# lukasc-ch/CBinfer

Measured on AMD Instinct MI355X. Metric: frames/sec + effective GFLOP/s vs dense, scene-labeling CNN 480x320 @10% change, higher is better.
Workload: dtype f32-equivalent: f32 tensors, every operand as three bf16 terms (24 bits, exact), six products on the bf16 MFMA, f32 accumulate; 1 GPU; sceneLabeling CBConv2d coarse-grained fp32, synthetic 480x320 seq @10% change (32x32 re-drawn blocks), experiment 6, one sequence per GPU; sequences_per_gpu=1, launch=program

## Files before the change

### cbinfer_amd/_lib.py

```python
import ctypes
import os

_PKG = os.path.dirname(os.path.abspath(__file__))
LIB_PATH = os.path.join(_PKG, "libcbinfer_hip.so")

CB_F32 = 0
CB_F16 = 1
CB_F32S = 2

_vp, _i, _l, _f = ctypes.c_void_p, ctypes.c_int, ctypes.c_long, ctypes.c_float


class SplitSeq(ctypes.Structure):
    _fields_ = [("input", _vp), ("state", _vp), ("splitState", _vp), ("frameMasks", _vp), ("producerMask", _vp),
                ("output", _vp), ("idxOut", _vp), ("countOut", _vp), ("rangeFlag", _vp), ("maskCopy", _vp),
                ("delta", _vp), ("reluOut", _vp)]


_sp = ctypes.POINTER(SplitSeq)


class TailSeq(ctypes.Structure):
    _fields_ = [("input", _vp), ("changeList", _vp), ("countDev", _vp), ("output", _vp)]

# ... 146 lines not shown
    "cbinfer_rowconv_prep_weights": (_i, [_vp, _vp, _i, _i, _i, _i, _vp]),
    "cbinfer_conv_changed_rows": (_i, [_vp, _vp, _vp, _vp, _vp, _vp, _vp, _i, _i, _i, _i, _i, _i, _i, _vp]),
    "cbinfer_change_detection_bits_pooled": (_i, [_vp, _i, _i, _vp, _vp, _vp, _i, _i, _i, _i, _i, _f, _i, _vp]),
    "cbinfer_cbconv2d_forward_rows": (_i, [_vp, _vp, _i, _i, _vp, _vp, _vp, _vp, _vp, _vp, _vp, _vp, _i, _i, _i,
                                           _i, _i, _i, _f, _i, _i, _i, _vp]),
    "cbinfer_cbconv2d_forward_blocks": (_i, [_vp, _vp, _i, _i, _vp, _vp, _vp, _vp, _vp, _vp, _vp, _vp, _i, _i,
                                             _i, _i, _i, _i, _f, _i, _i, _i, _vp]),
    "cbinfer_blockconv_supported": (_i, [_i, _i, _i, _i]),
    "cbinfer_blockconv_prepared_bytes": (_l, [_i, _i, _i, _i]),
    "cbinfer_blockconv_prep_weights": (_i, [_vp, _vp, _i, _i, _i, _i, _vp]),
    "cbinfer_conv_changed_blocks": (_i, [_vp, _vp, _vp, _vp, _vp, _vp, _vp, _i, _i, _i, _i, _i, _i, _i, _vp]),
    "cbinfer_change_detection_bits_batched": (_i, [_vpp, _vpp, _vpp, _i, _i, _i, _i, _i, _i, _f, _i, _vp]),
    "cbinfer_conv_changed_rows_batched": (_i, [_vpp, _vpp, _vpp, _vpp, _vpp, _i, _vp, _vp, _i, _i, _i, _i, _i, _i, _i,
                                               _vp]),
    "cbinfer_tail1x1_batched": (_i, [_tp, _i, _i, _vp, _vp, _vp, _vp, _i, _i, _i, _i, _i, _i, _i, _vp]),
    "cbinfer_split_supported": (_i, [_i, _i, _i, _i]),
    "cbinfer_split_max_sequences": (_i, []),
    "cbinfer_split_max_mask_words": (_l, [_i]),
    "cbinfer_split_state_bytes": (_l, [_i, _i, _i, _i, _i]),
    "cbinfer_split_prepared_bytes": (_l, [_i, _i, _i, _i]),
    "cbinfer_split_workspace_bytes": (_l, [_i, _i, _i, _i, _i, _i, _i]),
    "cbinfer_split_prep_weights": (_i, [_vp, _vp, _i, _i, _i, _i, _i, _i, _f, _vp]),
    "cbinfer_split_state_init": (_i, [_vp, _i, _i, _i, _i, _i, _vp]),
    "cbinfer_split_state_rebuild": (_i, [_vp, _vp, _i, _i, _i, _i, _i, _vp, _vp]),
    "cbinfer_split3_state_bytes": (_l, [_i, _i, _i, _i, _i]),
    "cbinfer_split3_prepared_bytes": (_l, [_i, _i, _i, _i]),
    "cbinfer_split3_prep_weights": (_i, [_vp, _vp, _i, _i, _i, _i, _i, _i, _vp]),
    "cbinfer_split3_state_init": (_i, [_vp, _i, _i, _i, _i, _i, _vp]),
    "cbinfer_split3_state_rebuild": (_i, [_vp, _vp, _i, _i, _i, _i, _i, _vp]),
    "cbinfer_split_detect": (_i, [_sp, _i, _i, _i, _i, _i, _i, _i, _i, _i, _f, _vp]),
    "cbinfer_split_conv": (_i, [_sp, _i, _vp, _vp, _i, _i, _i, _i, _i, _i, _f, _i, _vp, _i, _vp]),
    "cbinfer_split_forward": (_i, [_sp, _i, _i, _i, _i, _vp, _vp, _i, _i, _i, _i, _i, _i, _f, _f, _i, _vp, _vp]),
    "cbinfer_split_next_supported": (_i, [_i, _i, _i, _i, _i, _i, _ndp]),
    "cbinfer_split_conv_next": (_i, [_sp, _i, _vp, _vp, _i, _i, _i, _i, _i, _i, _f, _i, _vp, _ndp, _vp]),
    "cbinfer_split_refresh_supported": (_i, [_i, _i, _i, _i, _i, _i]),
    "cbinfer_split_conv_refresh": (_i, [_sp, _i, _vp, _vp, _i, _i, _i, _i, _i, _i, _f, _i, _vp, _srp, _vp]),
    "cbinfer_split_conv_next_refresh": (_i, [_sp, _i, _vp, _vp, _i, _i, _i, _i, _i, _i, _f, _i, _vp, _ndp, _srp, _vp]),
    "cbinfer_split_forward_next": (_i, [_sp, _i, _i, _i, _i, _vp, _vp, _i, _i, _i, _i, _i, _i, _f, _f, _i, _vp, _ndp,
                                        _vp]),
    "cbinfer_split_forward_fg": (_i, [_sp, _i, _i, _i, _i, _vp, _i, _i, _i, _i, _i, _i, _f, _f, _vp, _vp]),
    "cbinfer_hsplit_supported": (_i, [_i, _i, _i, _i]),
    "cbinfer_hsplit_max_mask_words": (_l, [_i]),
    "cbinfer_hsplit_state_bytes": (_l, [_i, _i, _i, _i, _i]),
    "cbinfer_hsplit_prepared_bytes": (_l, [_i, _i, _i, _i]),
    "cbinfer_hsplit_workspace_bytes": (_l, [_i, _i, _i, _i, _i, _i]),
    "cbinfer_hsplit_prep_weights": (_i, [_vp, _vp, _i, _i, _i, _i, _i, _i, _vp]),
    "cbinfer_hsplit_state_init": (_i, [_vp, _i, _i, _i, _i, _i, _vp]),
    "cbinfer_hsplit_state_rebuild": (_i, [_vp, _vp, _i, _i, _i, _i, _i, _vp]),
    "cbinfer_hsplit_forward": (_i, [_vp, _vp, _i, _i, _i, _vp, _vp, _vp, _vp, _vp, _vp, _vp, _vp, _vp, _vp, _i, _i, _i,
                                    _i, _i, _i, _f, _i, _i, _vp, _vp]),
    "cbinfer_hsplit_group_workspace_bytes": (_l, [_i, _i, _i, _i, _i, _i, _i]),
    "cbinfer_hsplit_forward_group": (_i, [_hlp, _i, _i, _i, _i, _i, _i, _i, _i, _i, _i, _vp, _vp]),
    "cbinfer_split_forward_tail": (_i, [_sp, _i, _i, _i, _i, _vp, _vp, _i, _i, _i, _i, _i, _i, _f, _f, _i, _vp, _i,
                                        _stp, _vp]),
    "cbinfer_split_forward_fg_tail": (_i, [_sp, _i, _i, _i, _i, _vp, _i, _i, _i, _i, _i, _i, _f, _f, _vp, _stp, _vp]),
    "cbinfer_split_tail_supported": (_i, [_i, _i, _i, _i, _i, _i]),
    "cbinfer_split_conv_tail": (_i, [_sp, _i, _vp, _vp, _i, _i, _i, _i, _i, _i, _f, _i, _vp, _i, _stp, _vp]),
    "cbinfer_rowpairs_supported": (_i, [_i, _i, _i, _i, _i, _i]),
    "cbinfer_conv_changed_rowpairs": (_i, [_vp, _vp, _vp, _vp, _vp, _vp, _vp, _i, _i, _i, _i, _i, _i, _i, _ndp, _vp]),
    "cbinfer_conv_changed_rowpairs_batched": (_i, [_psp, _i, _vp, _vp, _i, _i, _i, _i, _i, _i, _i, _ndp, _vp]),
    "cbinfer_conv_rowpairs_detect": (_i, [_vp, _vp, _vp, _vp, _vp, _vp, _i, _i, _i, _i, _i, _i, _f, _i, _ndp, _vp]),
    "cbinfer_refresh_state": (_i, [_vp, _vp, _i, _i, _i, _f, _vp]),
    "cbinfer_cbconv2d_forward_rowpairs": (_i, [_vp, _vp, _vp, _vp, _vp, _vp, _vp, _vp, _i, _i, _i, _i, _i, _i, _f, _i,
                                               _ndp, _vp]),
    "cbinfer_frame_mask_copy_offset": (_l, [_i, _i]),
    "cbinfer_concat_channels": (_i, [_vpp, ctypes.POINTER(ctypes.c_int32), _i, _vp, _l, _i, _vp]),
# ... 124 lines not shown
```

### cbinfer_amd/csrc/cb_split.hip

```cpp
#include <stdlib.h>

#include <type_traits>

#include "cb_common.h"

#ifdef CBS_STAMP
__device__ unsigned long long cbs_stamp_buf[4 * 2048 * 16];
#define CB_TAIL_STAMP(i)                                                                 \
    do {                                                                                 \
        if (threadIdx.x == 0 && blockIdx.x < 2048)                                       \
            cbs_stamp_buf[(2 * 2048 + blockIdx.x) * 16 + (i)] = __builtin_amdgcn_s_memrealtime(); \
    } while (0)
#define CBS_DET_STAMP(i)                                                                                            \
    do {                                                                                                            \
        const unsigned wg = blockIdx.y * gridDim.x + blockIdx.x;                                                    \
        if (POOL && threadIdx.x == 0 && blockIdx.z == 0 && wg < 2048)                                               \
            cbs_stamp_buf[(3 * 2048 + wg) * 16 + (i)] = __builtin_amdgcn_s_memrealtime();                            \
    } while (0)
#else
#define CBS_DET_STAMP(i)
#endif
#include "cb_tail_core.h"
#include "cb_split_common.h"

// ... 266 lines not shown
#define CBH_NEXT CBINFER_HNEXT_MAX
struct CbhNext {
    _Float16* state;
    char* S;
    unsigned long long* masks;
    int kHH, kWH, Wp, rec, padY, padXL;
    float th;
    int pad_;
};
struct CbhLayer {
    const char* A;
    const _Float16* bias;
    int K, relu, nNext, pad_;
    CbhNext next[CBH_NEXT];
};
struct CbhExt {
    CbhLayer L[CBH_GROUP];
    int slabCap1;
    int pad_;
};
struct CbsNoExt {};
struct CbsWinExt {
    float* nstate;
    char* nS;
    unsigned long long* nmasks;
    int* nflag;
    int H2, W2, wpr2, kHH, kWH, Wp, rec, padY, padXL, planes;
    float th;
    unsigned long long magicW2;
    const float* sideFrame;
    float* sideState;
    int sideC, sideHW;
    float sideTh;
};
template <int AR>
struct CbsExtOf {
    typedef CbsNoExt type;
};
template <>
struct CbsExtOf<1> {
    typedef CbhExt type;
};
template <>
struct CbsExtOf<3> {
    typedef CbsWinExt type;
};
struct CbsSideExt {
    const float* sideFrame;
    float* sideState;
    int sideC, sideHW;
    float sideTh;
};
template <>
struct CbsExtOf<4> {
    typedef CbsSideExt type;
};

__device__ __forceinline__ void cbh_or_dilated(unsigned long long* masks, int y, int x, int H, int W, int wpr, int kHH,
                                               int kWH) {
    const int lo = max(x - kWH, 0), hi = min(x + kWH, W - 1);
    const int w0 = lo >> 6, w1 = hi >> 6;
    const unsigned long long m0 = (~0ull << (lo & 63)) & (w1 == w0 ? (~0ull >> (63 - (hi & 63))) : ~0ull);
    const unsigned long long m1 = ~0ull >> (63 - (hi & 63));
    for (int yy = max(y - kHH, 0); yy <= min(y + kHH, H - 1); ++yy) {
        atomicOr(&masks[(long)yy * wpr + w0], m0);
        if (w1 != w0) atomicOr(&masks[(long)yy * wpr + w1], m1);
// ... 27 lines not shown

template <int OFF>
__device__ __forceinline__ halfx8 cbs_lds_read16(unsigned addr) {
    halfx8 v;
    asm volatile("ds_read_b128 %0, %1 offset:%2" : "=v"(v) : "v"(addr), "n"(OFF));
    return v;
}

__device__ __forceinline__ int cbs_div(int x, unsigned long long magic) {
    return (int)(((unsigned long long)(unsigned)x * magic) >> 32);
}

template <int BM, int BN, int WM, int WN, int PRE_CAP, bool MASK_LDS, int RING, int AR = 0>
__global__ __launch_bounds__(64 * WM * WN) void cbs_conv_kernel(CbsParams p, typename CbsExtOf<AR>::type ext) {
    constexpr bool HALF = AR == 1, X3 = AR == 2 || AR == 3 || AR == 4, WIN = AR == 3, SIDE = AR == 3 || AR == 4;
    if (HALF && p.upstream && *p.upstream == 0) {
        if (blockIdx.x == 0 && threadIdx.x == 0) {
            p.seq[0].countOut[0] = 0;
            if (p.info) p.info[CBS_INFO_SK] = 1;
        }
        return;
    }
    cb_touch_kernarg<sizeof(CbsParams) + (HALF ? sizeof(CbhExt) : (WIN ? sizeof(CbsWinExt) : (SIDE ? sizeof(CbsSideExt) : 0)))>();
    constexpr int NW = WM * WN, NT = 64 * NW;
    constexpr int TN = BN / WN / 32;
    static_assert(BM == 32 * WM, "one 32-row tile per wave");
    constexpr int PB = X3 ? 192 : 128;
    constexpr int ABLK = BM * PB / 1024, BBLK = BN * PB / 1024;
    constexpr int APW = ABLK / NW, BPW = BBLK / NW;
    static_assert(APW * NW == ABLK && BPW * NW == BBLK && APW >= 1 && BPW >= 1, "DMA blocks must deal evenly");
    constexpr int DPW = APW + BPW;
    constexpr int A_BYTES = BM * PB, B_BYTES = BN * PB, STAGE = A_BYTES + B_BYTES;
    constexpr int TILE = BM * BN;
    __shared__ __attribute__((aligned(1024))) char ring[RING * STAGE];
    __shared__ int s_pre[PRE_CAP + 1];
    __shared__ unsigned long long s_mask[MASK_LDS ? PRE_CAP : 1];
    __shared__ const unsigned long long* s_maskPtr[CBS_MAXSEQ];
    __shared__ int s_wsum[NW];
    __shared__ int s_tilePix[BN];
    __shared__ float s_bias[BM];
    __shared__ unsigned s_nchg[HALF ? CBH_NEXT * (BN / 32) : 1];
    __shared__ int s_preW[WIN ? PRE_CAP / 2 + 2 : 1];
    __shared__ int s_tileAny[WIN ? BN : 1];
    __shared__ int s_winPos[WIN ? BN / 4 : 1];
    __shared__ unsigned s_wchg;
    __shared__ unsigned long long s_wsum64[WIN ? 64 * WM * WN / 64 : 1];
    static_assert(!WIN || (BN / WN / 32 == 1 && MASK_LDS), "window order: one column tile per wave, the mask words in LDS");

    const int t = threadIdx.x;
    const int lane = t & 63, wave = __builtin_amdgcn_readfirstlane(t >> 6);
    const int wm = wave % WM, wn = wave / WM;
    const int l31 = lane & 31, h = lane >> 5;
    const int MW = p.maskWords, MT = p.KP / BM;
#ifdef CBS_STAMP
    bool cbs_first = true;
#endif
    CBS_STAMP_AT(0);
    CBS_STAMP_AT(6);

    __shared__ int s_seqN[CBS_MAXSEQ], s_seqRank[CBS_MAXSEQ], s_seqTile[CBS_MAXSEQ + 1], s_exact[CBS_MAXSEQ];
    int flagv = 0;
    static_assert(NT >= CBS_MAXSEQ, "one thread per sequence");
    if (p.nSeq == 1) {
        if (t == 0) {
            const int* rf = p.seq[0].rangeFlag;
            s_maskPtr[0] = p.seq[0].masks;
            if (rf) flagv = *rf;
// ... 252 lines not shown
        p.info[CBS_INFO_SK] = SK;
        p.info[CBS_INFO_MT] = MT;
        p.info[2] = p.nSeq;
        for (int q = 0; q < CBS_MAXSEQ; ++q) {
            p.info[CBS_INFO_TP + q] = q < p.nSeq ? s_seqTile[q + 1] - s_seqTile[q] : 0;
            p.info[CBS_INFO_TP + CBS_MAXSEQ + q] = q < p.nSeq ? s_seqN[q] : 0;
        }
        if constexpr (HALF) {
#pragma unroll
            for (int u = 0; u < CBH_GROUP; ++u) p.info[CBS_INFO_CH + u] = chQ[u];
        }
    }

    const int aRecords = (int)min(p.aBytes, (long)0x7fffffff);
    const cb_const_int* stageOff = (const cb_const_int*)p.stageOff;
    const int HW = p.H * p.W;
    const float lo2 = 1.0f / CBS_LO;

    static_assert(APW == (X3 ? 3 : 2) && BPW == APW, "four (x3: six) DMA instructions per wave and stage");
    int aRead[4];
#pragma unroll
    for (int e = 0; e < 4; ++e) {
        const int b = wm * 4 + e;
        aRead[e] = X3 ? (2 * wm) * 6144 + lane * 16 : (b / APW) * 4096 + (b % APW) * 1024 + lane * 16;
    }
    int bRead[TN];
#pragma unroll
    for (int j = 0; j < TN; ++j) {
        const int n = (wn * TN + j) * 32 + l31, c = n >> 3;
        if (X3)
            bRead[j] = (n >> 4) * 6144 + 3072 + (n & 15) * 64 + ((h ^ ((n >> 2) & 3)) << 4);
        else
            bRead[j] = (c / BPW) * 4096 + (APW + c % BPW) * 1024 + (n & 7) * 128 + ((h ^ ((n >> 1) & 7)) << 4);
    }

    for (int it = blockIdx.x; it < items; it += gridDim.x) {
        int d = cbs_div(it, p.magicMT), mt = it - d * MT;
        int slice = d & (SK - 1), ptg = SK == 1 ? d : d >> chShift;
        int q = 0, N = totAll, rb = 0, tile0 = 0;
        int CHi = CH, chShiftI = chShift;
        if constexpr (HALF) {
            static_assert(CBH_GROUP == 2, "two item ranges");
            q = (p.nSeq > 1 && it >= itemBase[1]) ? 1 : 0;
            const int local = it - (q ? itemBase[1] : 0);
            CHi = q ? chQ[CBH_GROUP - 1] : chQ[0];
            chShiftI = CHi >= 16 ? 4 : (CHi >= 8 ? 3 : 2);
            d = cbs_div(local, p.magicMT), mt = local - d * MT;
            slice = SK == 1 ? 0 : d & (CHi - 1);
            ptg = SK == 1 ? d : d >> chShiftI;
            if (p.nSeq > 1) {
                N = __builtin_amdgcn_readfirstlane(s_seqN[q]), rb = __builtin_amdgcn_readfirstlane(s_seqRank[q]);
            }
        } else if (p.nSeq > 1) {
            for (int u = 1; u < p.nSeq; ++u)
                if (ptg >= s_seqTile[u]) q = u;
            q = __builtin_amdgcn_readfirstlane(q);
            N = __builtin_amdgcn_readfirstlane(s_seqN[q]), rb = __builtin_amdgcn_readfirstlane(s_seqRank[q]);
            tile0 = __builtin_amdgcn_readfirstlane(s_seqTile[q]);
        }
        const int n0 = (ptg - tile0) * BN, m0 = mt * BM;
        const char* Aq = p.A;
        const float* biasq = p.bias;
        int Kq = p.K, reluq = p.relu, nNext = 0;
        if constexpr (HALF) {
            Aq = ext.L[q].A, biasq = (const float*)ext.L[q].bias, Kq = ext.L[q].K, reluq = ext.L[q].relu;
            nNext = __builtin_amdgcn_readfirstlane(ext.L[q].nNext);
// ... 410 lines not shown
        typedef std::integral_constant<int, 8> R8;
#define CBS_STEP3A(S, FCUR, FNEXT)                                                         \
        do {                                                                               \
            CBS_SB();                                                                      \
            mma3(KS0(), FCUR, 0, 1); CBS_SB(); read1(KS1(), P0(), (S), FNEXT); read1(KS1(), P3(), (S), FNEXT); CBS_SB(); \
            mma3(KS0(), FCUR, 1, 2); CBS_SB(); read1(KS1(), P1(), (S), FNEXT); read1(KS1(), P4(), (S), FNEXT); CBS_SB(); \
            mma3(KS0(), FCUR, 2, 3); CBS_SB(); read1(KS1(), P2t(), (S), FNEXT); read1(KS1(), P5(), (S), FNEXT); CBS_SB(); \
            mma3(KS0(), FCUR, 3, 4); CBS_SB(); read1(KS1(), R6(), (S), FNEXT); CBS_SB();   \
            mma3(KS0(), FCUR, 4, 5); CBS_SB(); read1(KS1(), R7(), (S), FNEXT); CBS_SB();   \
            mma3(KS0(), FCUR, 5, 6); CBS_SB(); read1(KS1(), R8(), (S), FNEXT); CBS_SB();   \
            mma3(KS0(), FCUR, 6, NM3);                                                     \
            waitFrags(FNEXT);                                                              \
        } while (0)
#define CBS_STEP3B(WAITN, S, FCUR, FNEXT)                                                  \
        do {                                                                               \
            asm volatile("s_waitcnt vmcnt(%0)" ::"n"(WAITN) : "memory");                  \
            __builtin_amdgcn_s_barrier();                                                  \
            CBS_SB();                                                                      \
            issue((S) + RING, true);                                                       \
            CBS_SB();                                                                      \
            mma3(KS1(), FCUR, 0, 1); CBS_SB();                                             \
            read1(KS0(), P0(), (S) + 1, FNEXT); read1(KS0(), P3(), (S) + 1, FNEXT); CBS_SB(); issuePart(P0()); CBS_SB(); \
            mma3(KS1(), FCUR, 1, 2); CBS_SB();                                             \
            read1(KS0(), P1(), (S) + 1, FNEXT); read1(KS0(), P4(), (S) + 1, FNEXT); CBS_SB(); issuePart(P1()); CBS_SB(); \
            mma3(KS1(), FCUR, 2, 3); CBS_SB();                                             \
            read1(KS0(), P2t(), (S) + 1, FNEXT); read1(KS0(), P5(), (S) + 1, FNEXT); CBS_SB(); issuePart(P2t()); CBS_SB(); \
            mma3(KS1(), FCUR, 3, 4); CBS_SB(); read1(KS0(), R6(), (S) + 1, FNEXT); CBS_SB(); issuePart(P3()); CBS_SB(); \
            mma3(KS1(), FCUR, 4, 5); CBS_SB(); read1(KS0(), R7(), (S) + 1, FNEXT); CBS_SB(); issuePart(P4()); CBS_SB(); \
            mma3(KS1(), FCUR, 5, 6); CBS_SB(); read1(KS0(), R8(), (S) + 1, FNEXT); CBS_SB(); issuePart(P5()); CBS_SB(); \
            mma3(KS1(), FCUR, 6, NM3);                                                     \
            waitFrags(FNEXT);                                                              \
        } while (0)

        constexpr bool NEXT_REGS = HALF && TN == 1;
        _Float16 hv16[NEXT_REGS ? 16 : 1], sv16[NEXT_REGS ? CBH_NEXT : 1][NEXT_REGS ? 16 : 1];
        if constexpr (NEXT_REGS) {
            if (nNext > 0 && SK == 1) {
                const int pixLd = max(s_tilePix[wn * 32 + l31], 0);
                const int nx2 = nNext > 1 ? 1 : 0;
                const int mb0 = m0 + wm * 32 + 4 * h;
#pragma unroll
                for (int r = 0; r < 16; ++r) {
                    const long o = (long)min(mb0 + 8 * (r >> 2) + (r & 3), Kq - 1) * HW + pixLd;
                    sv16[0][r] = ext.L[q].next[0].state[o];
                    if (CBH_NEXT > 1) sv16[CBH_NEXT > 1 ? 1 : 0][r] = ext.L[q].next[nx2].state[o];
                }
            }
        }
        float oldv[WIN ? 16 : 1], nsv[WIN ? 4 : 1];
        int anyPos = -1, wPos = -1;
        if constexpr (WIN) {
            const int nl = wn * 32 + l31;
            anyPos = s_tileAny[nl], wPos = s_winPos[nl >> 2];
            const int aLd = max(anyPos, 0), wLd = max(wPos, 0);
            const long H2W2 = (long)ext.H2 * ext.W2;
            const float* oq = p.seq[0].out;
            if (__builtin_amdgcn_ballot_w64(anyPos >= 0 && s_tilePix[nl] < 0) != 0ull) {
#pragma unroll
                for (int r = 0; r < 16; ++r) {
                    const int m = min(wm * 32 + (r & 3) + 8 * (r >> 2) + 4 * h, Kq - 1);
                    oldv[r] = oq[(long)m * HW + aLd];
                }
            } else {
#pragma unroll
                for (int r = 0; r < 16; ++r) oldv[r] = 0.f;
            }
            const int c0 = wm * 32 + 8 * (nl & 3) + 4 * h;
#pragma unroll
            for (int e = 0; e < 4; ++e) nsv[e] = ext.nstate[(long)min(c0 + e, Kq - 1) * H2W2 + wLd];
        }
        Frags F0, F1;
        CBS_STAMP_AT(2);
#pragma unroll
        for (int i = 0; i < RING; ++i) issue(sBeg + i);
        asm volatile("s_waitcnt vmcnt(%0)" ::"n"((RING - 1) * DPW) : "memory");
        __builtin_amdgcn_s_barrier();
        __builtin_amdgcn_sched_barrier(0);
        if constexpr (X3) {
            readA3(KS0(), sBeg, F0);
#pragma unroll
            for (int j = 0; j < TN; ++j) readB3(KS0(), sBeg, F0, j);
        } else {
            readFrags(sBeg, F0);
        }
        waitFrags(F0);
        if (t < BM) s_bias[t] = biasv;
        CBS_STAMP_AT(3);
        int s = sBeg;
        if constexpr (X3) {
            for (int c = c0; c < c1; ++c) {
                const int cEnd = chunkBeg(c + 1);
                for (; s < cEnd; ++s) {
                    CBS_STEP3A(s, F0, F1);
                    CBS_STEP3B((RING - 2) * DPW, s, F1, F0);
                }
                if (c + 1 < c1) fold();
            }
        }
        if constexpr (!X3) {
            for (int c = c0; c < c1; ++c) {
                const int cEnd = chunkBeg(c + 1);
                for (; s + 1 < cEnd; s += 2) {
                    CBS_STEP((RING - 2) * DPW, true, s, F0, F1);
                    CBS_STEP((RING - 2) * DPW, true, s + 1, F1, F0);
                }
                if (c + 1 < c1) fold();
            }
            if (s < sEnd) CBS_STEP((RING - 2) * DPW, true, s, F0, F1);
        }
        asm volatile("s_waitcnt vmcnt(0)" ::: "memory");
#undef CBS_STEP
#undef CBS_STEP3A
#undef CBS_STEP3B
#undef CBS_SB
        __builtin_amdgcn_sched_barrier(0);
        CBS_STAMP_AT(4);
        CBS_STAMP_AT(7);

        float* out = p.seq[q].out;
        int accum;
        float* reluPlane;
        {
            const char* ka = (const char*)__builtin_amdgcn_kernarg_segment_ptr();
            asm volatile("" : "+s"(ka));
            const CbsParams* pp = (const CbsParams*)ka;
            accum = pp->accumulate;
            reluPlane = accum ? pp->seq[q].reluOut : nullptr;
        }
        if (CBS_DBGBIT(32)) continue;
        if (SK > 1) {
            float4* slab = (float4*)p.slabs + (long)it * (TILE / 4);
#pragma unroll
            for (int j = 0; j < TN; ++j) {
                const int nl = (wn * TN + j) * 32 + l31;
#pragma unroll
                for (int r4 = 0; r4 < 4; ++r4) {
                    const int mq = wm * 8 + 2 * r4 + h;
                    slab[mq * BN + nl] = make_float4(comb(j, 4 * r4), comb(j, 4 * r4 + 1), comb(j, 4 * r4 + 2),
                                                     comb(j, 4 * r4 + 3));
                }
            }
            CBS_STAMP_AT(5);
#ifdef CBS_STAMP
            cbs_first = false;
// ... 746 lines not shown
        CB_REQUIRE(seqs[q].input && seqs[q].state && seqs[q].splitState && seqs[q].frameMasks);
        a.seq[q].in = seqs[q].input;
        a.seq[q].state = seqs[q].state;
        a.seq[q].S = (char*)seqs[q].splitState;
        a.seq[q].masks = (unsigned long long*)seqs[q].frameMasks;
        a.seq[q].prodMask = (pooled && !fg) ? (const unsigned long long*)seqs[q].producerMask : nullptr;
        a.seq[q].rangeFlag = x3 ? nullptr : seqs[q].rangeFlag;
        a.seq[q].delta = seqs[q].delta;
        if (fg) CB_REQUIRE(seqs[q].delta != nullptr);
    }
    a.W = W, a.H = H, a.C = C, a.kHH = (kH - 1) / 2, a.kWH = (kW - 1) / 2;
    a.wpr = cbinfer_mask_words_per_row(W), a.pH = pH, a.pW = pW;
    a.Wp = g.Wp, a.rec = g.rec, a.padY = g.padY, a.padXL = g.padXL;
    a.words = cbinfer_mask_words(H, W);
    a.th = threshold;
    a.copyAll = ((mode >> 1) & 1) | fg;
    a.fg = fg;
    dim3 grid(a.wpr, H, nSeq), block(64 * (C / 4));
    if (pooled)
        hipLaunchKernelGGL(cbs_detect_kernel<true>, grid, block, 0, (hipStream_t)stream, a);
    else
        hipLaunchKernelGGL(cbs_detect_kernel<false>, grid, block, 0, (hipStream_t)stream, a);
    return cb_launch_status();
}

static int cbs_detect_mode(int mode, float weightScale) {
    return (mode & ~CBINFER_SPLIT_X3) | (weightScale == 0.f ? CBINFER_SPLIT_X3 : 0);
}

static bool cbs_next_supported(int C, int K, int kH, int kW, int H, int W, const cbNextDetect* next) {
    if (!next || !cbs_supported(C, K, kH, kW) || K > 64 || K % 16 != 0 || !cbs_supported(K, 1, next->kH, next->kW)) return false;
    if (cbs_geom(C, H, W, kH, kW, 3).nStages >= 48) return false;
    if (!((next->H == H / 2 || next->H == (H + 1) / 2) && (next->W == W / 2 || next->W == (W + 1) / 2))) return false;
    if (next->arith != 0 && next->arith != 1) return false;
    const long MW = cbinfer_mask_words(H, W), EU = (long)((H + 1) / 2) * cbinfer_mask_words_per_row(W);
    if (MW > CBS_PRE_SMALL || 2 * EU + 2 > CBS_PRE_SMALL + 1 || EU + 1 > CBS_PRE_SMALL / 2 + 2) return false;
    const CbsGeom g2 = cbs_geom(K, next->H, next->W, next->kH, next->kW, next->arith ? 3 : 2);
    return (long)g2.Hp * g2.Wp * g2.rec < (1l << 31) && (long)H * W < (1l << 20);
}

static bool cbs_refresh_supported(int C, int K, int kH, int kW, int H, int W) {
    return cbs_supported(C, K, kH, kW) && K <= 64 && cbs_geom(C, H, W, kH, kW, 3).nStages < 48 &&
           cbinfer_mask_words(H, W) <= CBS_PRE_SMALL;
}

static int cbs_split_conv(const cbSplitSeq* seqs, int nSeq, const void* prepared, const float* bias, int C, int H,
                          int W, int K, int kH, int kW, float weightScale, int relu, void* workspace, int forceSplit,
                          const CbsTailArgs* tail, cbStream_t stream, int accumulate = 0,
                          const cbNextDetect* next = nullptr, const cbSideRefresh* side = nullptr) {
    if (workspace == nullptr && cbs_supported(C, K, kH, kW) && cbs_geom(C, H, W, kH, kW).nStages >= 48)
        return CB_ERR_BADARG;
    CB_REQUIRE(seqs && nSeq >= 1 && nSeq <= CBS_MAXSEQ && prepared && H > 0 && W > 0 && weightScale >= 0.f);
    if (!cbs_supported(C, K, kH, kW)) return CB_ERR_UNSUPPORTED;
    const bool x3 = weightScale == 0.f;
    const CbsGeom g = cbs_geom(C, H, W, kH, kW, x3 ? 3 : 2);
    const int KP = cbs_kp(K), BM = cbs_bm(K);
    const long MW = cbinfer_mask_words(H, W);
    if ((long)nSeq * MW > (BM >= 128 ? CBS_PRE_BIG : CBS_PRE_MID) || (long)g.Hp * g.Wp * g.rec >= (1l << 31) ||
        (long)H * W * W >= (1l << 32))
        return CB_ERR_UNSUPPORTED;
    CbsParams p;
    for (int q = 0; q < nSeq; ++q) {
        CB_REQUIRE(seqs[q].splitState && seqs[q].output && seqs[q].frameMasks && seqs[q].idxOut && seqs[q].countOut);
        p.seq[q].S = (const char*)seqs[q].splitState;
        p.seq[q].state = accumulate ? seqs[q].delta : seqs[q].state;
        p.seq[q].reluOut = accumulate ? seqs[q].reluOut : nullptr;
        p.seq[q].rangeFlag = (p.seq[q].state && !x3) ? seqs[q].rangeFlag : nullptr;
        p.seq[q].out = seqs[q].output;
        p.seq[q].masks = (unsigned long long*)seqs[q].frameMasks;
        p.seq[q].listOut = seqs[q].idxOut;
        p.seq[q].countOut = seqs[q].countOut;
        p.seq[q].maskCopy = (unsigned long long*)seqs[q].maskCopy;
    }
    p.nSeq = nSeq;
    p.aBytes = (long)g.nStages * (KP / 32) * (x3 ? 6144 : 4096);
    p.A = (const char*)prepared;
    p.stageOff = (const int*)((const char*)prepared + p.aBytes);
    p.wPlain = x3 ? nullptr : (const float*)((const char*)prepared + cbs_plain_offset(p.aBytes, g.nStages));
    p.bias = bias;
    p.relu = relu;
    cbs_fill_params(p, g, K, KP, BM, H, W, MW, workspace, cbs_slab_capacity(nSeq, H, W, K));
    p.outScale = x3 ? 1.0f : 1.0f / (weightScale * CBS_XSCALE);
    p.forceSK = forceSplit;
    p.accumulate = accumulate;
    p.halfOut = 0;
    p.upstream = nullptr;
    p.maxChunks = CBS_CHUNKS;
#ifdef CBS_DBG
    if (const char* e = getenv("CBINFER_SPLIT_DBG")) p.dbg = atoi(e);
#endif
    hipStream_t s = (hipStream_t)stream;
    if (side && side->frame && !next) {
        if (!cbs_refresh_supported(C, K, kH, kW, H, W) || nSeq != 1 || !x3 || accumulate || tail) return CB_ERR_UNSUPPORTED;
        CbsSideExt e;
        const int st = cbs_fill_side(e, side);
        if (st != CB_OK) return st;
        return cbs_launch_conv<64, 64, 2, 2, CBS_PRE_SMALL, true, 5, 4>(p, 1, nullptr, s, e);
    }
    if (next) {
        if (!cbs_next_supported(C, K, kH, kW, H, W, next) || nSeq != 1 || !x3 || accumulate || tail) return CB_ERR_UNSUPPORTED;
        CB_REQUIRE(next->state && next->splitState && next->frameMasks);
        const CbsGeom g2 = cbs_geom(K, next->H, next->W, next->kH, next->kW, next->arith ? 3 : 2);
        CbsWinExt e;
        e.nstate = next->state, e.nS = (char*)next->splitState, e.nmasks = (unsigned long long*)next->frameMasks;
        e.nflag = next->arith ? nullptr : next->rangeFlag;
        e.H2 = next->H, e.W2 = next->W, e.wpr2 = cbinfer_mask_words_per_row(next->W);
        e.kHH = (next->kH - 1) / 2, e.kWH = (next->kW - 1) / 2;
        e.Wp = g2.Wp, e.rec = g2.rec, e.padY = g2.padY, e.padXL = g2.padXL, e.planes = g2.planes;
        e.th = next->threshold;
        e.magicW2 = (1ull << 32) / (unsigned long long)next->W + 1ull;
        e.sideFrame = nullptr, e.sideState = nullptr, e.sideC = 0, e.sideHW = 0, e.sideTh = 0.f;
        if (side && side->frame) {
            const int st = cbs_fill_side(e, side);
            if (st != CB_OK) return st;
        }
        return cbs_launch_conv<64, 64, 2, 2, CBS_PRE_SMALL, true, 5, 3>(p, 1, nullptr, s, e);
    }
    if (x3) {
        if (BM == 128) {
            if ((long)nSeq * MW <= CBS_PRE_X3) return cbs_launch_conv<128, 128, 4, 2, CBS_PRE_X3, true, 3, 2>(p, 1, tail, s);
            return cbs_launch_conv<128, 128, 4, 2, CBS_PRE_BIG, false, 3, 2>(p, 1, tail, s);
        }
        if (nSeq == 1 && MW <= CBS_PRE_SMALL) return cbs_launch_conv<64, 64, 2, 2, CBS_PRE_SMALL, true, 5, 2>(p, 1, tail, s);
        if ((long)nSeq * MW <= CBS_PRE_SMALL) return cbs_launch_conv<64, 64, 2, 2, CBS_PRE_SMALL, false, 3, 2>(p, 2, tail, s);
        return cbs_launch_conv<64, 64, 2, 2, CBS_PRE_MID, false, 5, 2>(p, 1, tail, s);
    }
    if (BM == 128) return cbs_launch_conv<128, 128, 4, 2, CBS_PRE_BIG, true, 4>(p, 1, tail, s);
    if (nSeq == 1 && MW <= CBS_PRE_SMALL) return cbs_launch_conv<64, 64, 2, 2, CBS_PRE_SMALL, true, 8>(p, 1, tail, s);
    if ((long)nSeq * MW <= CBS_PRE_SMALL) return cbs_launch_conv<64, 64, 2, 2, CBS_PRE_SMALL, true, 4>(p, 2, tail, s);
    if ((long)nSeq * MW <= CBS_PRE_MID2) return cbs_launch_conv<64, 64, 2, 2, CBS_PRE_MID2, false, 4>(p, 2, tail, s);
    return cbs_launch_conv<64, 64, 2, 2, CBS_PRE_MID, false, 3>(p, 2, tail, s);
}

int cbinfer_split_conv(const cbSplitSeq* seqs, int nSeq, const void* prepared, const float* bias, int C, int H,
                       int W, int K, int kH, int kW, float weightScale, int relu, void* workspace, int forceSplit,
                       cbStream_t stream) {
    return cbs_split_conv(seqs, nSeq, prepared, bias, C, H, W, K, kH, kW, weightScale, relu, workspace, forceSplit,
                          nullptr, stream);
}

int cbinfer_split_tail_supported(int C, int K, int kH, int kW, int C1, int C2) {
    return cbs_supported(C, K, kH, kW) && cbs_geom(C, 64, 64, kH, kW).nStages >= 48 && K % 16 == 0 && C1 >= 4 && C2 >= 1 &&
           C1 <= 16 * CB_TAIL_MAXW && cb_tail_lds_bytes(K, C1, C2) <= 60 * 1024;
}
// ... 31 lines not shown
    const int st = cbinfer_split_detect(seqs, nSeq, cbs_detect_mode(mode, weightScale), pH, pW, C, H, W, kH, kW, threshold,
                                        stream);
    if (st != CB_OK) return st;
    return cbinfer_split_conv_tail(seqs, nSeq, prepared, bias, C, H, W, K, kH, kW, weightScale, relu, workspace,
                                   forceSplit, tail, stream);
}

int cbinfer_split_forward_fg(const cbSplitSeq* seqs, int nSeq, int pooled, int pH, int pW, const void* prepared, int C,
                             int H, int W, int K, int kH, int kW, float threshold, float weightScale, void* workspace,
                             cbStream_t stream) {
    const int st = cbinfer_split_detect(seqs, nSeq,
                                        cbs_detect_mode(CBINFER_SPLIT_FG | (pooled ? CBINFER_SPLIT_POOLED : 0), weightScale),
                                        pH, pW, C, H, W, kH, kW, threshold, stream);
    if (st != CB_OK) return st;
    return cbs_split_conv(seqs, nSeq, prepared, nullptr, C, H, W, K, kH, kW, weightScale, 0, workspace, 0, nullptr,
                          stream, 1);
}

int cbinfer_split_forward_fg_tail(const cbSplitSeq* seqs, int nSeq, int pooled, int pH, int pW, const void* prepared,
                                  int C, int H, int W, int K, int kH, int kW, float threshold, float weightScale,
                                  void* workspace, const cbSplitTail* tail, cbStream_t stream) {
    CbsTailArgs ta;
    int st = cbs_tail_args(ta, tail, nSeq, nullptr, C, K, kH, kW);
    if (st != CB_OK) return st;
    st = cbinfer_split_detect(seqs, nSeq, cbs_detect_mode(CBINFER_SPLIT_FG | (pooled ? CBINFER_SPLIT_POOLED : 0), weightScale),
                              pH, pW, C, H, W, kH, kW, threshold, stream);
    if (st != CB_OK) return st;
    return cbs_split_conv(seqs, nSeq, prepared, nullptr, C, H, W, K, kH, kW, weightScale, 0, workspace, 0, &ta,
                          stream, 1);
}

int cbinfer_split_next_supported(int C, int K, int kH, int kW, int H, int W, const cbNextDetect* next) {
    return cbs_next_supported(C, K, kH, kW, H, W, next) ? 1 : 0;
}
int cbinfer_split_conv_next(const cbSplitSeq* seqs, int nSeq, const void* prepared, const float* bias, int C, int H,
                            int W, int K, int kH, int kW, float weightScale, int relu, void* workspace,
                            const cbNextDetect* next, cbStream_t stream) {
    CB_REQUIRE(next);
    return cbs_split_conv(seqs, nSeq, prepared, bias, C, H, W, K, kH, kW, weightScale, relu, workspace, 0, nullptr, stream,
                          0, next);
}
int cbinfer_split_conv_next_refresh(const cbSplitSeq* seqs, int nSeq, const void* prepared, const float* bias, int C, int H,
                                    int W, int K, int kH, int kW, float weightScale, int relu, void* workspace,
                                    const cbNextDetect* next, const cbSideRefresh* side, cbStream_t stream) {
    CB_REQUIRE(next && side);
    return cbs_split_conv(seqs, nSeq, prepared, bias, C, H, W, K, kH, kW, weightScale, relu, workspace, 0, nullptr, stream,
                          0, next, side);
}
int cbinfer_split_refresh_supported(int C, int K, int kH, int kW, int H, int W) {
    return cbs_refresh_supported(C, K, kH, kW, H, W) ? 1 : 0;
}
int cbinfer_split_conv_refresh(const cbSplitSeq* seqs, int nSeq, const void* prepared, const float* bias, int C, int H, int W,
                               int K, int kH, int kW, float weightScale, int relu, void* workspace,
                               const cbSideRefresh* side, cbStream_t stream) {
    CB_REQUIRE(side && side->frame);
    return cbs_split_conv(seqs, nSeq, prepared, bias, C, H, W, K, kH, kW, weightScale, relu, workspace, 0, nullptr, stream,
                          0, nullptr, side);
}
int cbinfer_split_forward_next(const cbSplitSeq* seqs, int nSeq, int mode, int pH, int pW, const void* prepared,
                               const float* bias, int C, int H, int W, int K, int kH, int kW, float threshold,
                               float weightScale, int relu, void* workspace, const cbNextDetect* next,
                               cbStream_t stream) {
    CB_REQUIRE(next);
    if (!cbs_next_supported(C, K, kH, kW, H, W, next) || nSeq != 1 || weightScale != 0.f) return CB_ERR_UNSUPPORTED;
    const int st = cbinfer_split_detect(seqs, nSeq, cbs_detect_mode(mode, weightScale), pH, pW, C, H, W, kH, kW, threshold,
                                        stream);
// ... 402 lines not shown
```

### include/cbinfer_hip.h

```cpp
#ifndef CBINFER_HIP_H
#define CBINFER_HIP_H

#include <stdint.h>

#ifdef __cplusplus
extern "C" {
#endif

typedef void* cbStream_t;

#define CB_F32 0
#define CB_F16 1
#define CB_F32S 2

#define CB_OK 0
#define CB_ERR_BADARG (-1)
#define CB_ERR_UNSUPPORTED (-2)

#define CBINFER_ABI_VERSION 11

int cbinfer_abi_version(void);
const char* cbinfer_status_string(int status);

int cbinfer_mask_words_per_row(int W);
// ... 279 lines not shown
    const int32_t* upstreamCount;
    const void* input;
    const uint64_t* producerMask;
    void* state;
    void* pixelState;
    uint64_t* frameMasks;
    void* output;
    int32_t* idxOut;
    int32_t* countOut;
    uint64_t* maskCopy;
    const void* prepared;
    const void* bias;
    int K;
    float threshold;
    int relu;
    int detect;
    int nNext;
    int reserved;
    cbHalfNext next[CBINFER_HNEXT_MAX];
} cbHalfLayer;
long cbinfer_hsplit_group_workspace_bytes(int nLayers, int C, int H, int W, int K, int kH, int kW);
int cbinfer_hsplit_forward_group(const cbHalfLayer* layers, int nLayers, int pooled, int pH, int pW, int C, int H, int W,
                                 int kH, int kW, int feedbackLoop, void* workspace, cbStream_t stream);

typedef struct {
    float* state;
    void* splitState;
    uint64_t* frameMasks;
    int32_t* rangeFlag;
    int H, W, kH, kW;
    float threshold;
    int arith;
} cbNextDetect;
typedef struct {
    const float* state;
    float* output;
    uint64_t* bits;
    uint64_t* maskCopy;
    float* nextState;
    void* nextSplitState;
    uint64_t* nextFrameMasks;
    int32_t* nextRangeFlag;
} cbPairSeq;
int cbinfer_rowpairs_supported(int C, int K, int kH, int kW, int H, int W);
int cbinfer_conv_changed_rowpairs_batched(const cbPairSeq* seqs, int nSeq, const void* prepared, const float* bias,
                                          int C, int H, int W, int K, int kH, int kW, int relu,
                                          const cbNextDetect* next, cbStream_t stream);
int cbinfer_conv_rowpairs_detect(const float* input, const float* prevInput, float* prevOutput, uint64_t* maskCopy,
                                 const void* prepared, const float* bias, int C, int H, int W, int K, int kH, int kW,
                                 float threshold, int relu, const cbNextDetect* next, cbStream_t stream);
int cbinfer_refresh_state(const float* frame, float* state, int C, int H, int W, float threshold, cbStream_t stream);
int cbinfer_conv_changed_rowpairs(const float* state, uint64_t* bits, int32_t* ctl, uint64_t* maskCopy,
                                  const void* prepared, const float* bias, float* output, int C, int H, int W, int K,
                                  int kH, int kW, int relu, const cbNextDetect* next, cbStream_t stream);
int cbinfer_cbconv2d_forward_rowpairs(const float* input, float* prevInput, float* prevOutput, uint64_t* bits,
                                      int32_t* ctl, uint64_t* maskCopy, const void* prepared, const float* bias, int C,
                                      int H, int W, int K, int kH, int kW, float threshold, int relu,
                                      const cbNextDetect* next, cbStream_t stream);

typedef struct {
    const float* frame;
    float* state;
    int C, H, W;
    float threshold;
} cbSideRefresh;
int cbinfer_split_conv_next_refresh(const cbSplitSeq* seqs, int nSeq, const void* prepared, const float* bias, int C, int H,
                                    int W, int K, int kH, int kW, float weightScale, int relu, void* workspace,
                                    const cbNextDetect* next, const cbSideRefresh* side, cbStream_t stream);
int cbinfer_split_refresh_supported(int C, int K, int kH, int kW, int H, int W);
int cbinfer_split_conv_refresh(const cbSplitSeq* seqs, int nSeq, const void* prepared, const float* bias, int C, int H, int W,
                               int K, int kH, int kW, float weightScale, int relu, void* workspace,
                               const cbSideRefresh* side, cbStream_t stream);
int cbinfer_split_next_supported(int C, int K, int kH, int kW, int H, int W, const cbNextDetect* next);
int cbinfer_split_conv_next(const cbSplitSeq* seqs, int nSeq, const void* prepared, const float* bias, int C, int H,
                            int W, int K, int kH, int kW, float weightScale, int relu, void* workspace,
                            const cbNextDetect* next, cbStream_t stream);
int cbinfer_split_forward_next(const cbSplitSeq* seqs, int nSeq, int mode, int pH, int pW, const void* prepared,
                               const float* bias, int C, int H, int W, int K, int kH, int kW, float threshold,
                               float weightScale, int relu, void* workspace, const cbNextDetect* next,
                               cbStream_t stream);

#define CBINFER_CONCAT_MAX 4
int cbinfer_concat_channels(const void* const* sources, const int32_t* channels, int n, void* output, long HW, int dtype,
                            cbStream_t stream);

typedef struct cbGeom {
    int kH, kW, sH, sW, pH, pW, dH, dW;
} cbGeom;
int cbinfer_geom_out_size(int Hi, int Wi, const cbGeom* geom, int* Ho, int* Wo);
long cbinfer_geom_prepared_weights_bytes(int K, int C, const cbGeom* geom, int dtype);
int cbinfer_geom_prep_weights(const void* weight, void* prepared, int K, int C, int Hi, int Wi, const cbGeom* geom,
                              int dtype, cbStream_t stream);
long cbinfer_geom_workspace_bytes(void);
int cbinfer_change_detection_geom(const void* input, void* state, uint64_t* frameMasks, int C, int Hi, int Wi,
                                  const cbGeom* geom, float threshold, int updateInputState, int dtype,
                                  cbStream_t stream);
int cbinfer_conv_changed_geom(const void* input, const int32_t* changeList, int numChanges, const int32_t* countDev,
                              uint64_t* frameMasks, int32_t* idxOut, int32_t* countOut, const void* prepared,
                              const void* bias, void* output, int C, int Hi, int Wi, int K, const cbGeom* geom, int relu,
                              void* workspace, int dtype, cbStream_t stream);
int cbinfer_cbconv2d_forward_geom(const void* input, void* prevInput, void* prevOutput, uint64_t* frameMasks,
                                  int32_t* idx, int32_t* countDev, const void* prepared, const void* bias, int C, int Hi,
                                  int Wi, int K, const cbGeom* geom, float threshold, int feedbackLoop, int copyInput,
                                  int relu, int haveIndexes, int capN, void* workspace, int dtype, cbStream_t stream);

#define CB_POOL_MAX 0
// ... 82 lines not shown
```

Before: 11510 frames/s.

## Stage input patches once per window in LDS and stream only weights

```diff
diff --git a/cbinfer_amd/_lib.py b/cbinfer_amd/_lib.py
--- a/cbinfer_amd/_lib.py
+++ b/cbinfer_amd/_lib.py
@@ -202,6 +202,7 @@
     "cbinfer_split_conv": (_i, [_sp, _i, _vp, _vp, _i, _i, _i, _i, _i, _i, _f, _i, _vp, _i, _vp]),
     "cbinfer_split_forward": (_i, [_sp, _i, _i, _i, _i, _vp, _vp, _i, _i, _i, _i, _i, _i, _f, _f, _i, _vp, _vp]),
     "cbinfer_split_next_supported": (_i, [_i, _i, _i, _i, _i, _i, _ndp]),
+    "cbinfer_split_next_patch_form": (_i, [_i, _i, _i, _i, _i, _i, _ndp]),
     "cbinfer_split_conv_next": (_i, [_sp, _i, _vp, _vp, _i, _i, _i, _i, _i, _i, _f, _i, _vp, _ndp, _vp]),
     "cbinfer_split_refresh_supported": (_i, [_i, _i, _i, _i, _i, _i]),
     "cbinfer_split_conv_refresh": (_i, [_sp, _i, _vp, _vp, _i, _i, _i, _i, _i, _i, _f, _i, _vp, _srp, _vp]),
diff --git a/cbinfer_amd/csrc/cb_split.hip b/cbinfer_amd/csrc/cb_split.hip
--- a/cbinfer_amd/csrc/cb_split.hip
+++ b/cbinfer_amd/csrc/cb_split.hip
@@ -322,6 +322,11 @@
     float* sideState;
     int sideC, sideHW;
     float sideTh;
+    int patchRow;
+    int patchBytes;
+    int patchNI;
+    int patchSpr;
+    unsigned long long magicPRow;
 };
 template <int AR>
 struct CbsExtOf {
@@ -415,7 +420,10 @@
     constexpr int DPW = APW + BPW;
     constexpr int A_BYTES = BM * PB, B_BYTES = BN * PB, STAGE = A_BYTES + B_BYTES;
     constexpr int TILE = BM * BN;
-    __shared__ __attribute__((aligned(1024))) char ring[RING * STAGE];
+    constexpr int PR = 3, P_WMAX = 6144, P_WSTRIDE = P_WMAX + 64, P_WOFF = ((BN / 4) * P_WSTRIDE + 64 + 1023) / 1024 * 1024;
+    constexpr int P_TOTAL = P_WOFF + PR * A_BYTES;
+    constexpr int RING_BYTES = (WIN && P_TOTAL > RING * STAGE) ? P_TOTAL : RING * STAGE;
+    __shared__ __attribute__((aligned(1024))) char ring[RING_BYTES];
     __shared__ int s_pre[PRE_CAP + 1];
     __shared__ unsigned long long s_mask[MASK_LDS ? PRE_CAP : 1];
     __shared__ const unsigned long long* s_maskPtr[CBS_MAXSEQ];
@@ -734,6 +742,23 @@
             bRead[j] = (n >> 4) * 6144 + 3072 + (n & 15) * 64 + ((h ^ ((n >> 2) & 3)) << 4);
         else
             bRead[j] = (c / BPW) * 4096 + (APW + c % BPW) * 1024 + (n & 7) * 128 + ((h ^ ((n >> 1) & 7)) << 4);
+    }
+
+    int pRel[P_WMAX / 1024];
+    bool patchOn = false;
+    if constexpr (WIN) {
+        patchOn = ext.patchRow != 0;
+        if (patchOn) {
+#pragma unroll
+            for (int i = 0; i < P_WMAX / 1024; ++i) {
+                int b = i * 1024 + lane * 16;
+                if (b >= ext.patchBytes) b -= ext.patchBytes;
+                const int R = cbs_div(b, ext.magicPRow), o = b - R * ext.patchRow;
+                pRel[i] = CBS_SPAD + R * (p.Wp * p.rec) + (o ^ ((R & 1) << 4));
+            }
+            if (t < 8 * (BN / 4))
+                *(uint4*)(ring + (t >> 3) * P_WSTRIDE + ext.patchNI * 1024 + (t & 7) * 16) = make_uint4(0u, 0u, 0u, 0u);
+        }
     }
 
     for (int it = blockIdx.x; it < items; it += gridDim.x) {
@@ -1210,6 +1235,39 @@
             waitFrags(FNEXT);                                                              \
         } while (0)
 
+#define CBS_STEP3A_P(S, FCUR, FNEXT)                                                       \
+        do {                                                                               \
+            const unsigned so_ = (unsigned)(((S) % PR) * A_BYTES);                         \
+            CBS_SB();                                                                      \
+            mma3(KS0(), FCUR, 0, 1); CBS_SB(); read1P(KS1(), P0(), so_, bCur, FNEXT); read1P(KS1(), P3(), so_, bCur, FNEXT); CBS_SB(); \
+            mma3(KS0(), FCUR, 1, 2); CBS_SB(); read1P(KS1(), P1(), so_, bCur, FNEXT); read1P(KS1(), P4(), so_, bCur, FNEXT); CBS_SB(); \
+            mma3(KS0(), FCUR, 2, 3); CBS_SB(); read1P(KS1(), P2t(), so_, bCur, FNEXT); read1P(KS1(), P5(), so_, bCur, FNEXT); CBS_SB(); \
+            mma3(KS0(), FCUR, 3, NM3);                                                     \
+            waitFrags(FNEXT);                                                              \
+        } while (0)
+#define CBS_STEP3B_P(WAITN, S, FCUR, FNEXT)                                                \
+        do {                                                                               \
+            asm volatile("s_waitcnt vmcnt(%0)" ::"n"(WAITN) : "memory");                  \
+            __builtin_amdgcn_s_barrier();                                                  \
+            CBS_SB();                                                                      \
+            issueP((S) + PR, true);                                                        \
+            const unsigned so_ = (unsigned)((((S) + 1) % PR) * A_BYTES);                   \
+            {                                                                              \
+                const bool wrap_ = pSc + 1 == ext.patchSpr;                                \
+                pSc = wrap_ ? 0 : pSc + 1;                                                 \
+                bCur = (bCur + (wrap_ ? ext.patchRow - (ext.patchSpr - 1) * 192 : 192)) ^ (wrap_ ? 16u : 0u); \
+            }                                                                              \
+            CBS_SB();                                                                      \
+            mma3(KS1(), FCUR, 0, 1); CBS_SB();                                             \
+            read1P(KS0(), P0(), so_, bCur, FNEXT); read1P(KS0(), P3(), so_, bCur, FNEXT); CBS_SB(); issuePart(P0()); CBS_SB(); \
+            mma3(KS1(), FCUR, 1, 2); CBS_SB();                                             \
+            read1P(KS0(), P1(), so_, bCur, FNEXT); read1P(KS0(), P4(), so_, bCur, FNEXT); CBS_SB(); issuePart(P1()); CBS_SB(); \
+            mma3(KS1(), FCUR, 2, 3); CBS_SB();                                             \
+            read1P(KS0(), P2t(), so_, bCur, FNEXT); read1P(KS0(), P5(), so_, bCur, FNEXT); CBS_SB(); issuePart(P2t()); CBS_SB(); \
+            mma3(KS1(), FCUR, 3, NM3);                                                     \
+            waitFrags(FNEXT);                                                              \
+        } while (0)
+
         constexpr bool NEXT_REGS = HALF && TN == 1;
         _Float16 hv16[NEXT_REGS ? 16 : 1], sv16[NEXT_REGS ? CBH_NEXT : 1][NEXT_REGS ? 16 : 1];
         if constexpr (NEXT_REGS) {
@@ -1247,8 +1305,69 @@
 #pragma unroll
             for (int e = 0; e < 4; ++e) nsv[e] = ext.nstate[(long)min(c0 + e, Kq - 1) * H2W2 + wLd];
         }
+        const unsigned pwBase = ringBase + P_WOFF + wm * 6144 + lane * 16;
+        unsigned bCur = 0;
+        int pSc = 0;
+        auto issueP = [&](int s, bool setUpOnly = false) {
+            const bool live = s < sEnd;
+            const int aS = live ? s * aStageBytes + aItem : 0;
+            const __amdgpu_buffer_rsrc_t ar = __builtin_amdgcn_make_buffer_rsrc((void*)Aq, 0, live ? aRecords : 0, 0x00020000);
+            char* mine = ring + P_WOFF + (s % PR) * A_BYTES + wave * (APW * 1024);
+            if (setUpOnly) {
+                isA = ar, isMine = mine, isAS = aS;
+                return;
+            }
+            cbs_dma16<0>(ar, mine, aVoff, aS);
+            cbs_dma16<1024>(ar, mine, aVoff, aS);
+            cbs_dma16<2048>(ar, mine, aVoff, aS);
+        };
+        auto read1P = [&](auto ksTag, auto rTag, unsigned so, unsigned bA, Frags& f) {
+            constexpr int KS = decltype(ksTag)::value, R = decltype(rTag)::value;
+            if constexpr (R < 3)
+                f.a[R] = cbs_lds_read16<(3 * KS + R) * 1024>(pwBase + so);
+            else
+                f.b[R - 3] = cbs_lds_read16<KS * 96 + (R - 3) * 32>(bA);
+        };
         Frags F0, F1;
         CBS_STAMP_AT(2);
+        bool patchDone = false;
+        if constexpr (WIN) {
+          if (patchOn) {
+            patchDone = true;
+            {
+                const __amdgpu_buffer_rsrc_t br = __builtin_amdgcn_make_buffer_rsrc((void*)Sq, 0, bRecords, 0x00020000);
+                const int rowB = p.Wp * p.rec;
+#pragma unroll
+                for (int j = 0; j < BN / 4 / NW; ++j) {
+                    const int r = wave * (BN / 4 / NW) + j;
+                    const int a0 = __builtin_amdgcn_readfirstlane(s_tileAny[4 * r]);
+                    const int py = cbs_div(max(a0, 0), p.magicW);
+                    const int base = a0 < 0 ? p.dummyBase - rowB : (py * p.Wp + (a0 - py * p.W)) * p.rec;
+                    char* dst = ring + r * P_WSTRIDE;
+#pragma unroll
+                    for (int i = 0; i < P_WMAX / 1024; ++i)
+                        if (i < ext.patchNI) cbs_dma16<0>(br, dst + i * 1024, pRel[i], base);
+                }
+                const int nl = wn * 32 + l31, dy = (nl >> 1) & 1;
+                bCur = ringBase + (nl >> 2) * P_WSTRIDE + dy * ext.patchRow + (nl & 1) * p.rec + (((h ^ dy) & 1) << 4);
+            }
+#pragma unroll
+            for (int i = 0; i < PR; ++i) issueP(sBeg + i);
+            asm volatile("s_waitcnt vmcnt(%0)" ::"n"((PR - 1) * APW) : "memory");
+            __builtin_amdgcn_s_barrier();
+            __builtin_amdgcn_sched_barrier(0);
+            read1P(KS0(), P0(), 0u, bCur, F0), read1P(KS0(), P1(), 0u, bCur, F0), read1P(KS0(), P2t(), 0u, bCur, F0);
+            read1P(KS0(), P3(), 0u, bCur, F0), read1P(KS0(), P4(), 0u, bCur, F0), read1P(KS0(), P5(), 0u, bCur, F0);
+            waitFrags(F0);
+            if (t < BM) s_bias[t] = biasv;
+            CBS_STAMP_AT(3);
+            for (int s = sBeg; s < sEnd; ++s) {
+                CBS_STEP3A_P(s, F0, F1);
+                CBS_STEP3B_P((PR - 2) * APW, s, F1, F0);
+            }
+          }
+        }
+        if (!patchDone) {
 #pragma unroll
         for (int i = 0; i < RING; ++i) issue(sBeg + i);
         asm volatile("s_waitcnt vmcnt(%0)" ::"n"((RING - 1) * DPW) : "memory");
@@ -1286,8 +1405,11 @@
             }
             if (s < sEnd) CBS_STEP((RING - 2) * DPW, true, s, F0, F1);
         }
+        }
         asm volatile("s_waitcnt vmcnt(0)" ::: "memory");
 #undef CBS_STEP
+#undef CBS_STEP3A_P
+#undef CBS_STEP3B_P
 #undef CBS_STEP3A
 #undef CBS_STEP3B
 #undef CBS_SB
@@ -2100,11 +2222,18 @@
     if (!next || !cbs_supported(C, K, kH, kW) || K > 64 || K % 16 != 0 || !cbs_supported(K, 1, next->kH, next->kW)) return false;
     if (cbs_geom(C, H, W, kH, kW, 3).nStages >= 48) return false;
     if (!((next->H == H / 2 || next->H == (H + 1) / 2) && (next->W == W / 2 || next->W == (W + 1) / 2))) return false;
-    if (next->arith != 0 && next->arith != 1) return false;
+    const int arith = next->arith & ~CBINFER_NEXT_RING_OPERAND;
+    if (arith != 0 && arith != 1) return false;
     const long MW = cbinfer_mask_words(H, W), EU = (long)((H + 1) / 2) * cbinfer_mask_words_per_row(W);
     if (MW > CBS_PRE_SMALL || 2 * EU + 2 > CBS_PRE_SMALL + 1 || EU + 1 > CBS_PRE_SMALL / 2 + 2) return false;
-    const CbsGeom g2 = cbs_geom(K, next->H, next->W, next->kH, next->kW, next->arith ? 3 : 2);
+    const CbsGeom g2 = cbs_geom(K, next->H, next->W, next->kH, next->kW, arith ? 3 : 2);
     return (long)g2.Hp * g2.Wp * g2.rec < (1l << 31) && (long)H * W < (1l << 20);
+}
+
+static bool cbs_patch_form(int C, int K, int kH, int kW, int H, int W, const cbNextDetect* next) {
+    if (!cbs_next_supported(C, K, kH, kW, H, W, next) || (next->arith & CBINFER_NEXT_RING_OPERAND)) return false;
+    const long bytes = (long)(kH + 1) * (kW + 1) * cbs_geom(C, H, W, kH, kW, 3).rec;
+    return (bytes + 1023) / 1024 * 1024 <= 6144;
 }
 
 static bool cbs_refresh_supported(int C, int K, int kH, int kW, int H, int W) {
@@ -2168,16 +2297,23 @@
     if (next) {
         if (!cbs_next_supported(C, K, kH, kW, H, W, next) || nSeq != 1 || !x3 || accumulate || tail) return CB_ERR_UNSUPPORTED;
         CB_REQUIRE(next->state && next->splitState && next->frameMasks);
-        const CbsGeom g2 = cbs_geom(K, next->H, next->W, next->kH, next->kW, next->arith ? 3 : 2);
+        const int arith2 = next->arith & ~CBINFER_NEXT_RING_OPERAND;
+        const CbsGeom g2 = cbs_geom(K, next->H, next->W, next->kH, next->kW, arith2 ? 3 : 2);
         CbsWinExt e;
         e.nstate = next->state, e.nS = (char*)next->splitState, e.nmasks = (unsigned long long*)next->frameMasks;
-        e.nflag = next->arith ? nullptr : next->rangeFlag;
+        e.nflag = arith2 ? nullptr : next->rangeFlag;
         e.H2 = next->H, e.W2 = next->W, e.wpr2 = cbinfer_mask_words_per_row(next->W);
         e.kHH = (next->kH - 1) / 2, e.kWH = (next->kW - 1) / 2;
         e.Wp = g2.Wp, e.rec = g2.rec, e.padY = g2.padY, e.padXL = g2.padXL, e.planes = g2.planes;
         e.th = next->threshold;
         e.magicW2 = (1ull << 32) / (unsigned long long)next->W + 1ull;
         e.sideFrame = nullptr, e.sideState = nullptr, e.sideC = 0, e.sideHW = 0, e.sideTh = 0.f;
+        e.patchRow = 0, e.patchBytes = 0, e.patchNI = 0, e.patchSpr = 1, e.magicPRow = 0ull;
+        if (cbs_patch_form(C, K, kH, kW, H, W, next)) {
+            e.patchRow = (kW + 1) * g.rec, e.patchBytes = (kH + 1) * e.patchRow, e.patchNI = (e.patchBytes + 1023) / 1024;
+            e.patchSpr = g.pair ? g.kWs : kW * (g.G / 2);
+            e.magicPRow = (1ull << 32) / (unsigned long long)e.patchRow + 1ull;
+        }
         if (side && side->frame) {
             const int st = cbs_fill_side(e, side);
             if (st != CB_OK) return st;
@@ -2275,6 +2411,9 @@
 
 int cbinfer_split_next_supported(int C, int K, int kH, int kW, int H, int W, const cbNextDetect* next) {
     return cbs_next_supported(C, K, kH, kW, H, W, next) ? 1 : 0;
+}
+int cbinfer_split_next_patch_form(int C, int K, int kH, int kW, int H, int W, const cbNextDetect* next) {
+    return cbs_patch_form(C, K, kH, kW, H, W, next) ? 1 : 0;
 }
 int cbinfer_split_conv_next(const cbSplitSeq* seqs, int nSeq, const void* prepared, const float* bias, int C, int H,
                             int W, int K, int kH, int kW, float weightScale, int relu, void* workspace,
diff --git a/include/cbinfer_hip.h b/include/cbinfer_hip.h
--- a/include/cbinfer_hip.h
+++ b/include/cbinfer_hip.h
@@ -335,6 +335,7 @@
     float threshold;
     int arith;
 } cbNextDetect;
+#define CBINFER_NEXT_RING_OPERAND 0x100
 typedef struct {
     const float* state;
     float* output;
@@ -375,6 +376,7 @@
                                int K, int kH, int kW, float weightScale, int relu, void* workspace,
                                const cbSideRefresh* side, cbStream_t stream);
 int cbinfer_split_next_supported(int C, int K, int kH, int kW, int H, int W, const cbNextDetect* next);
+int cbinfer_split_next_patch_form(int C, int K, int kH, int kW, int H, int W, const cbNextDetect* next);
 int cbinfer_split_conv_next(const cbSplitSeq* seqs, int nSeq, const void* prepared, const float* bias, int C, int H,
                             int W, int K, int kH, int kW, float weightScale, int relu, void* workspace,
                             const cbNextDetect* next, cbStream_t stream);
```

Measured after the change: 11380 frames/s. 1.2% lower.
